# shenyunhang/JTSM

Hardware: AMD Instinct MI355X
Metric: images/sec training, R50-FPN JTSM panoptic, 2x1024x1024, 1/2/4/8 GPU (higher is better)
Workload: dtype bf16x3; 1 GPU; BASELINE configs[2]: JTSM panoptic R50-FPN, 2 x 3x1024x1024 per GPU, 2000 proposals + 1024 superpixels per image; MIL + 4 OICR + 2 mask heads + sem-seg; fwd + bwd + gradient exchange + SGD; 100% of proposals jittered copies of 40 rectangles per image; global_batch=2, parallelism=dp1, foreground_rois_last_step=281

## Files before the change

include/jtsm_hip.h:

```cpp
#ifndef JTSM_HIP_H_
#define JTSM_HIP_H_

#include <stddef.h>
#include <stdint.h>

#ifdef __cplusplus
extern "C" {
#endif

#define JTSM_OK 0
#define JTSM_EINVAL (-1)
#define JTSM_ELAUNCH (-2)
#define JTSM_ENODEV (-3)

#define JTSM_NCHW 0
#define JTSM_NHWC 1

const char* jtsm_last_error(void);
const char* jtsm_version(void);
int jtsm_device_count(void);

void* jtsm_event_create(void);
int jtsm_event_record(void* event, void* stream);
int jtsm_event_elapsed_ms(void* start, void* stop, float* ms);
// ... 73 lines not shown
                                        int sampling_ratio, int layout, void* workspace, size_t workspace_bytes,
                                        void* stream);
int jtsm_moi_pool_forward_f16(const uint16_t* input, const uint16_t* rois, const int32_t* oh_labels,
                              const int32_t* superpixels, uint16_t* output, int32_t* argmax, void* workspace,
                              size_t workspace_bytes, int B, int C, int H, int W, int M, int L, int Hs, int Ws,
                              float spatial_scale, int pooled_h, int pooled_w, int layout, void* stream);
int jtsm_moi_pool_backward_f16(const uint16_t* grad, const uint16_t* rois, const int32_t* argmax, uint16_t* grad_input,
                               void* workspace, size_t workspace_bytes, int B, int C, int H, int W, int M, int pooled_h,
                               int pooled_w, int layout, void* stream);

size_t jtsm_moi_pool_levels_workspace_bytes(int B, const int* H, const int* W, int nlevels, int M, int L);
int jtsm_moi_pool_forward_levels_f32(const float* const* inputs, const int* H, const int* W,
                                     const float* scales, int nlevels, const float* rois,
                                     const int32_t* roi_level, const int32_t* oh_labels,
                                     const int32_t* superpixels, float* output, int32_t* argmax,
                                     void* workspace, int B, int C, int M, int L, int Hs, int Ws,
                                     int pooled_h, int pooled_w, void* stream);
size_t jtsm_moi_pool_backward_levels_workspace_bytes(const int* H, const int* W, int nlevels, int B, int M);
int jtsm_moi_pool_backward_levels_f32(const float* grad, const float* rois, const int32_t* roi_level,
                                      const int32_t* argmax, float* const* grad_inputs, const int* H,
                                      const int* W, const float* scales, int nlevels, int B, int C, int M,
                                      int pooled_h, int pooled_w, int accumulate, void* workspace,
                                      size_t workspace_bytes, void* stream);

int jtsm_moi_mask_f32(const float* rois, const int32_t* oh_labels, const int32_t* superpixels,
                      int32_t* mois, void* workspace, int B, int H, int W, int M, int L, int Hs,
                      int Ws, float spatial_scale, void* stream);


typedef struct jtsm_conv_shape {
  int batch, in_h, in_w, in_c;
  int out_c;
  int kernel_h, kernel_w;
  int stride, pad, dilation;
} jtsm_conv_shape;

int jtsm_conv_out_size(const jtsm_conv_shape* s, int* out_h, int* out_w);
size_t jtsm_conv_workspace_bytes(const jtsm_conv_shape* s, int backward_data);
int jtsm_conv_plan(const jtsm_conv_shape* s, int role, int has_kscale, int* kernel, int* tile_m,
                   int* tile_n, int* splits);

int jtsm_conv2d_forward_f32(const float* x, const float* w, float* y, const jtsm_conv_shape* s,
                            const float* scale, const float* bias, const float* residual,
                            int relu, void* workspace, size_t workspace_bytes, void* stream);
int jtsm_conv2d_backward_data_f32(const float* dy, const float* w, float* dx,
                                  const jtsm_conv_shape* s, const float* kscale,
// ... 210 lines not shown

int jtsm_roi_align_forward_level_f32(const float* input, const float* rois,
                                     const int32_t* roi_level, int level, float* output, int B,
                                     int C, int H, int W, int M, float spatial_scale, int pooled_h,
                                     int pooled_w, int sampling_ratio, int aligned, void* stream);
int jtsm_roi_align_backward_level_f32(const float* grad, const float* rois,
                                      const int32_t* roi_level, int level, float* grad_input, int B,
                                      int C, int H, int W, int M, float spatial_scale, int pooled_h,
                                      int pooled_w, int sampling_ratio, int aligned, void* stream);
int jtsm_roi_align_rotated_forward_level_f32(const float* input, const float* rois, const int32_t* roi_level,
                                             int level, float* output, int B, int C, int H, int W, int M,
                                             float spatial_scale, int pooled_h, int pooled_w, int sampling_ratio,
                                             void* stream);
int jtsm_roi_align_rotated_backward_level_f32(const float* grad, const float* rois, const int32_t* roi_level,
                                              int level, float* grad_input, int B, int C, int H, int W, int M,
                                              float spatial_scale, int pooled_h, int pooled_w, int sampling_ratio,
                                              int accumulate, void* stream);
size_t jtsm_roi_align_backward_levels_workspace_bytes(const int* H, const int* W, int nlevels, int B, int C, int M);
int jtsm_roi_align_backward_levels_f32(const float* grad, const float* rois, const int32_t* roi_level,
                                       float* const* grad_inputs, const int* H, const int* W, const float* scales,
                                       int nlevels, int B, int C, int M, int pooled_h, int pooled_w, int sampling_ratio,
                                       int aligned, int accumulate, void* workspace, size_t workspace_bytes,
                                       void* stream);
int jtsm_moi_pool_forward_level_f32(const float* input, const float* rois, const int32_t* roi_level,
                                    int level, const int32_t* oh_labels, const int32_t* superpixels,
                                    float* output, int32_t* argmax, void* workspace, int B, int C,
                                    int H, int W, int M, int L, int Hs, int Ws, float spatial_scale,
                                    int pooled_h, int pooled_w, void* stream);
int jtsm_moi_pool_backward_level_f32(const float* grad, const float* rois, const int32_t* roi_level,
                                     int level, const int32_t* argmax, float* grad_input, int B, int C,
                                     int H, int W, int M, int pooled_h, int pooled_w, void* stream);


size_t jtsm_group_norm_workspace_bytes(int N, long HW, int C);
int jtsm_group_norm_forward_f32(const float* x, const float* gamma, const float* beta, float* y,
                                float* mean, float* rstd, void* workspace, int N, long HW, int C, int G,
                                float eps, int relu, void* stream);
int jtsm_group_norm_backward_f32(const float* x, const float* dy, const float* gamma, const float* beta,
                                 const float* mean, const float* rstd, float* dx, uint16_t* dx_hi,
                                 uint16_t* dx_lo, float* dgamma, float* dbeta, void* workspace, int N, long HW,
                                 int C, int G, int relu, void* stream);
int jtsm_upsample_bilinear2x_forward_f32(const float* x, float* y, uint16_t* y_hi, uint16_t* y_lo, int N, int H,
                                         int W, int C, void* stream);
int jtsm_upsample_bilinear2x_backward_f32(const float* gy, float* gx, int N, int H, int W, int C,
                                          void* stream);

// ... 78 lines not shown
```

jtsm_amd/csrc/moi_pool.hip:

```cpp
#include <algorithm>
#include <cfloat>

#include "common.h"

namespace jtsm {
namespace {

#pragma clang fp contract(off)

struct IBox { int b, x0, y0, x1, y1; };

__device__ __forceinline__ IBox round_box(const float* __restrict__ roi, float scale) {
#pragma clang fp contract(off)
  IBox r;
  r.b = (int)roi[0];
  r.x0 = (int)roundf(roi[1] * scale);
  r.y0 = (int)roundf(roi[2] * scale);
  r.x1 = (int)roundf(roi[3] * scale);
  r.y1 = (int)roundf(roi[4] * scale);
  return r;
}

__device__ __forceinline__ int clampi(int v, int lo, int hi) { return min(max(v, lo), hi); }

// ... 1273 lines not shown
static bool moi_bwd_events(hipEvent_t* fork, hipEvent_t* join) {
  static hipEvent_t ev[16][2] = {};
  int dev = 0;
  if (hipGetDevice(&dev) != hipSuccess || dev < 0 || dev >= 16) return false;
  for (int k = 0; k < 2; ++k)
    if (!ev[dev][k] && hipEventCreateWithFlags(&ev[dev][k], hipEventDisableTiming) != hipSuccess) return false;
  *fork = ev[dev][0];
  *join = ev[dev][1];
  return true;
}

static long census_tiles(const int* H, const int* W, int nlevels, int B) {
  long n = 0;
  for (int l = 0; l < nlevels; ++l) n += (long)B * ceil_div(W[l], kTile) * ceil_div(H[l], kTileY);
  return n;
}

size_t jtsm_moi_pool_backward_levels_workspace_bytes(const int* H, const int* W, int nlevels, int B, int M) {
  if (nlevels <= 0 || nlevels > kMaxLevels || B <= 0 || M <= 0 || !H || !W) return 0;
  return (((size_t)nlevels * B * ((size_t)M + 1) + 6 * (size_t)census_tiles(H, W, nlevels, B) + 8) * sizeof(int) + 15) &
         ~(size_t)15;
}

int jtsm_moi_pool_backward_levels_f32(const float* grad, const float* rois, const int32_t* roi_level,
                                      const int32_t* argmax, float* const* grad_inputs, const int* H, const int* W,
                                      const float* scales, int nlevels, int B, int C, int M, int pooled_h, int pooled_w,
                                      int accumulate, void* workspace, size_t workspace_bytes, void* stream) {
  JTSM_REQUIRE(nlevels > 0 && nlevels <= kMaxLevels && grad_inputs && H && W, "moi_pool levels backward: bad level table");
  JTSM_REQUIRE(B >= 0 && C >= 0 && M >= 0 && pooled_h > 0 && pooled_w > 0 && C % 4 == 0,
               "moi_pool levels backward: bad sizes (C %% 4 must be 0)");
  hipStream_t st = as_stream(stream);
  MoiLevels lv = {};
  bool all = true;
  for (int l = 0; l < nlevels; ++l) {
    lv.gin[l] = grad_inputs[l]; lv.H[l] = H[l]; lv.W[l] = W[l];
    lv.scale[l] = scales ? scales[l] : 0.f;
    all = all && grad_inputs[l] != nullptr;
  }
  bool small_maps = true;
  for (int l = 0; l < nlevels; ++l) small_maps = small_maps && (unsigned long long)H[l] * W[l] * W[l] < 0xFFFFFFFFull;
  const bool tiled = scales && workspace && all && small_maps && C % 256 == 0 && M > 0 && B > 0;
  if (tiled) {
    JTSM_REQUIRE(grad && rois && roi_level && argmax, "moi_pool levels backward: null pointer");
    const size_t need = jtsm_moi_pool_backward_levels_workspace_bytes(H, W, nlevels, B, M);
    JTSM_REQUIRE(workspace_bytes >= need && ((uintptr_t)workspace & 3) == 0,
                 "moi_pool levels backward: workspace of %zu bytes needed", need);
    int* lists = reinterpret_cast<int*>(workspace);
    int* counts = lists + (size_t)nlevels * B * M;
    int* census = counts + (size_t)nlevels * B;
    const int ntile = (int)census_tiles(H, W, nlevels, B);
    int* plan = census + ntile;
    hipLaunchKernelGGL(moi_roi_lists_kernel, dim3(nlevels * B), dim3(256), 0, st, rois, roi_level, M, B, lists, counts);
    MoiTiles tl = {};
    int blocks = 0;
    for (int l = 0; l < nlevels; ++l) {
      tl.first[l] = blocks;
      tl.tiles_x[l] = ceil_div(W[l], kTile);
      tl.tiles_y[l] = ceil_div(H[l], kTileY);
      blocks += B * tl.tiles_x[l] * tl.tiles_y[l];
    }
    tl.first[nlevels] = blocks;
    JTSM_CHECK_HIP(hipMemsetAsync(census, 0, (size_t)ntile * sizeof(int), st));
    hipLaunchKernelGGL(moi_tile_census_kernel, dim3(ceil_div(M, 256)), dim3(256), 0, st, lv, tl, rois, roi_level, M, nlevels,
                       pooled_h, pooled_w, census);
    int* tile_order = plan + 2 + 4 * (size_t)ntile;
    hipLaunchKernelGGL(tile_plan_kernel, dim3(1), dim3(1024), 0, st, census, ntile, plan, moi_heavy_min(), 4, tile_order);
    hipStream_t side = moi_bwd_side_stream();
    hipEvent_t fork = nullptr, join = nullptr;
    if (side && moi_bwd_events(&fork, &join)) {
      JTSM_CHECK_HIP(hipEventRecord(fork, st));
      JTSM_CHECK_HIP(hipStreamWaitEvent(side, fork, 0));
    } else {
      side = st;
    }
    hipLaunchKernelGGL(moi_pool_bwd_busy, dim3(256), dim3(1024), (size_t)kCopies * kQuad * kQuad * 256 * sizeof(float), side,
                       lv, tl, grad, rois, argmax, C, M, pooled_h, pooled_w, B, lists, counts, nlevels, plan, accumulate);
    hipLaunchKernelGGL(moi_pool_bwd_tiled, dim3(blocks, C / 256), dim3(256), kTile * kTile * 256 * sizeof(float), st, lv, tl,
                       grad, rois, argmax, C, M, pooled_h, pooled_w, B, lists, counts, nlevels, plan, census, moi_heavy_min(),
                       accumulate, tile_order);
    if (side != st) {
      JTSM_CHECK_HIP(hipEventRecord(join, side));
      JTSM_CHECK_HIP(hipStreamWaitEvent(st, join, 0));
    }
    hipLaunchKernelGGL(moi_pool_bwd_levels, dim3(std::min(ceil_div((long)M * pooled_h * pooled_w, 4), 8192)), dim3(256), 0,
                       st, lv, grad, rois, argmax, C, M, pooled_h * pooled_w, roi_level, nlevels, plan, kCensusLimit);
    JTSM_CHECK_LAUNCH("moi_pool backward levels (tiled)");
    return JTSM_OK;
  }
  for (int l = 0; l < nlevels; ++l) {
    if (!grad_inputs[l] || accumulate) continue;
    JTSM_CHECK_HIP(hipMemsetAsync(grad_inputs[l], 0, (size_t)B * H[l] * W[l] * C * sizeof(float), st));
  }
  if ((long)M * C == 0) return JTSM_OK;
  JTSM_REQUIRE(grad && rois && roi_level && argmax, "moi_pool levels backward: null pointer");
  for (int l = 0; l < nlevels; ++l)
    JTSM_REQUIRE(grad_inputs[l], "moi_pool levels backward: every level needs a gradient buffer");
  const int nbins = pooled_h * pooled_w;
  hipLaunchKernelGGL(moi_pool_bwd_levels, dim3(std::min(ceil_div((long)M * nbins, 4), 8192)), dim3(256), 0, st, lv, grad,
                     rois, argmax, C, M, nbins, roi_level, nlevels, (const int*)nullptr, 0);
  JTSM_CHECK_LAUNCH("moi_pool backward levels");
  return JTSM_OK;
}

}
```

jtsm_amd/csrc/roi_align.hip:

```cpp
#include <cstdlib>
#include <type_traits>

#include "common.h"
#include "roi_geometry.h"

namespace jtsm {
namespace {

#pragma clang fp contract(off)

template <typename T, int VEC> struct VecOf;
template <> struct VecOf<float, 4> { using type = float4; };
template <> struct VecOf<float, 1> { using type = float; };
template <> struct VecOf<double, 2> { using type = double2; };
template <> struct VecOf<double, 1> { using type = double; };

template <typename T, int VEC>
__device__ __forceinline__ void load_vec(const T* p, T (&v)[VEC]) {
  using V = typename VecOf<T, VEC>::type;
  const V x = *reinterpret_cast<const V*>(p);
  const T* e = reinterpret_cast<const T*>(&x);
#pragma unroll
  for (int i = 0; i < VEC; ++i) v[i] = e[i];
}
// ... 582 lines not shown
  } else {
    JTSM_REQUIRE(!roi_level, "roi_align: per-level filtering needs the NHWC layout");
    const long total = (long)M * C * PH * PW;
    const int blocks = (int)((total + 255) / 256 < 8192 ? (total + 255) / 256 : 8192);
    hipLaunchKernelGGL((align_fwd_nchw<T, ROT>), dim3(blocks), dim3(256), 0, st, in, rois, out, C,
                       H, W, total, scale, PH, PW, sr, aligned);
  }
  JTSM_CHECK_LAUNCH("roi_align forward");
  return JTSM_OK;
}

static size_t align_gather_head_bytes(int ntile, int C) {
  return ((size_t)ntile * (1 + C / 64) * sizeof(int) + 4 * sizeof(int) + 15) & ~(size_t)15;
}
static size_t align_gather_bytes(int ntile, int C, int M) {
  return align_gather_head_bytes(ntile, C) + (size_t)M * (sizeof(int4) + sizeof(int));
}
struct AsyncScratch {
  void* p = nullptr;
  hipStream_t st = nullptr;
  ~AsyncScratch() { if (p) (void)hipFreeAsync(p, st); }
};

static int align_backward_gather(const float* grad, const float* rois, AlignLevels& lv, int B, int C, int M, int PH,
                                 int PW, int sr, int aligned, const int* roi_level, hipStream_t st, bool accumulate = false,
                                 void* workspace = nullptr, size_t workspace_bytes = 0) {
  int ntile = 0;
  for (int l = 0; l < lv.n; ++l) {
    lv.tiles_x[l] = ceil_div(lv.W[l], kTile);
    lv.tiles_y[l] = ceil_div(lv.H[l], kTile);
    lv.first_tile[l] = ntile;
    ntile += B * lv.tiles_x[l] * lv.tiles_y[l];
  }
  lv.first_tile[lv.n] = ntile;
  const size_t need = align_gather_bytes(ntile, C, M);
  AsyncScratch own;
  own.st = st;
  if (workspace) {
    JTSM_REQUIRE(workspace_bytes >= need && ((uintptr_t)workspace & 15) == 0,
                 "roi_align backward: workspace of %zu bytes (16-byte aligned) needed, got %zu", need, workspace_bytes);
  } else {
    JTSM_CHECK_HIP(hipMallocAsync(&own.p, need, st));
  }
  for (int l = 0; l < lv.n && !accumulate; ++l)
    JTSM_CHECK_HIP(hipMemsetAsync(lv.gin[l], 0, (size_t)B * lv.H[l] * lv.W[l] * C * sizeof(float), st));
  int* census = reinterpret_cast<int*>(workspace ? workspace : own.p);
  const int fan = C / 64;
  const size_t head = align_gather_head_bytes(ntile, C);
  JTSM_CHECK_HIP(hipMemsetAsync(census, 0, (size_t)ntile * sizeof(int), st));
  int* plan = census + ntile;
  int4* reach = reinterpret_cast<int4*>(reinterpret_cast<char*>(census) + head);
  int* meta = reinterpret_cast<int*>(reach + M);
  hipLaunchKernelGGL(align_census_kernel, dim3(ceil_div(M, 256)), dim3(256), 0, st, rois, M, PH, PW, sr, aligned,
                     roi_level, lv, census, reach, meta);
  hipLaunchKernelGGL(tile_plan_kernel, dim3(1), dim3(1024), 0, st, census, ntile, plan, 1, fan);
  hipLaunchKernelGGL((align_bwd_gather<8, 1>), dim3(std::min(ntile * fan, 512)), dim3(256), 0, st, grad, rois, lv, C, M, PH,
                     PW, sr, aligned, plan, census_limit(), fan, reach, meta, accumulate ? 1 : 0);
  constexpr int V = WideVec<float>::value;
  const int blocks = ceil_div((long)M * PH * PW, 4);
  if (C % V == 0 && ((uintptr_t)grad % (V * sizeof(float))) == 0)
    hipLaunchKernelGGL((align_bwd_nhwc_levels<V>), dim3(blocks), dim3(256), 0, st, grad, rois, lv, C, M, PH, PW, sr, aligned,
                       roi_level, plan, census_limit());
  else
    hipLaunchKernelGGL((align_bwd_nhwc_levels<1>), dim3(blocks), dim3(256), 0, st, grad, rois, lv, C, M, PH, PW, sr, aligned,
                       roi_level, plan, census_limit());
  JTSM_CHECK_LAUNCH("roi_align backward (gather + census)");
  return JTSM_OK;
}

template <typename T, bool ROT>
int launch_backward(const T* grad, const T* rois, T* gin, int B, int C, int H, int W, int M,
                    T scale, int PH, int PW, int sr, int aligned, int layout, void* stream,
                    const int* roi_level = nullptr, int level = 0, bool accumulate = false) {
  JTSM_REQUIRE(B >= 0 && C >= 0 && H >= 0 && W >= 0 && M >= 0 && PH > 0 && PW > 0,
               "roi_align backward: negative size");
  JTSM_REQUIRE(layout == JTSM_NCHW || layout == JTSM_NHWC, "roi_align: unknown layout %d", layout);
  hipStream_t st = as_stream(stream);
  const size_t in_elems = (size_t)B * C * H * W;
  if (in_elems == 0) return JTSM_OK;
  JTSM_REQUIRE(gin, "roi_align backward: null grad_input");
// ... 366 lines not shown
                                             int level, float* output, int B, int C, int H, int W, int M,
                                             float spatial_scale, int pooled_h, int pooled_w, int sampling_ratio,
                                             void* stream) {
  JTSM_REQUIRE(roi_level || M == 0, "roi_align_rotated level: null roi_level");
  return launch_forward<float, true>(input, rois, output, B, C, H, W, M, spatial_scale, pooled_h, pooled_w,
                                     sampling_ratio, 1, JTSM_NHWC, stream, roi_level, level);
}
int jtsm_roi_align_rotated_backward_level_f32(const float* grad, const float* rois, const int32_t* roi_level,
                                              int level, float* grad_input, int B, int C, int H, int W, int M,
                                              float spatial_scale, int pooled_h, int pooled_w, int sampling_ratio,
                                              int accumulate, void* stream) {
  JTSM_REQUIRE(roi_level || M == 0, "roi_align_rotated level: null roi_level");
  return launch_backward<float, true>(grad, rois, grad_input, B, C, H, W, M, spatial_scale, pooled_h, pooled_w,
                                      sampling_ratio, 1, JTSM_NHWC, stream, roi_level, level, accumulate != 0);
}

size_t jtsm_roi_align_backward_levels_workspace_bytes(const int* H, const int* W, int nlevels, int B, int C, int M) {
  if (!H || !W || nlevels <= 0 || B <= 0 || C <= 0 || M < 0) return 0;
  long ntile = 0;
  for (int l = 0; l < nlevels; ++l) ntile += (long)B * ceil_div(W[l], kTile) * ceil_div(H[l], kTile);
  return align_gather_bytes((int)ntile, C, M);
}

int jtsm_roi_align_backward_levels_f32(const float* grad, const float* rois, const int32_t* roi_level,
                                       float* const* grad_inputs, const int* H, const int* W, const float* scales,
                                       int nlevels, int B, int C, int M, int pooled_h, int pooled_w, int sampling_ratio,
                                       int aligned, int accumulate, void* workspace, size_t workspace_bytes,
                                       void* stream) {
  JTSM_REQUIRE(nlevels > 0 && nlevels <= kAlignLevels && grad_inputs && H && W && scales,
               "roi_align levels: bad level table");
  JTSM_REQUIRE(B >= 0 && C >= 0 && M >= 0 && pooled_h > 0 && pooled_w > 0, "roi_align levels: negative size");
  JTSM_REQUIRE(roi_level || M == 0, "roi_align levels: null roi_level");
  hipStream_t st = as_stream(stream);
  const bool gather = C % 64 == 0 && C > 0 && B > 0 && grad && rois && pooled_w <= kMaxBins && pooled_h <= kMaxBins &&
                      (long)M * pooled_h * pooled_w >= 8192 && (long)M * pooled_h * pooled_w < (1L << 30);
  if (gather) {
    AlignLevels lv = {};
    lv.n = 0;
    for (int l = 0; l < nlevels; ++l) {
      if (!grad_inputs[l]) continue;
      JTSM_REQUIRE(H[l] > 0 && W[l] > 0, "roi_align levels: empty map");
      const int k = lv.n++;
      lv.gin[k] = grad_inputs[l]; lv.H[k] = H[l]; lv.W[k] = W[l]; lv.scale[k] = scales[l]; lv.level_id[k] = l;
    }
    if (lv.n == 0) return JTSM_OK;
    return align_backward_gather(grad, rois, lv, B, C, M, pooled_h, pooled_w, sampling_ratio, aligned, roi_level, st,
                                 accumulate != 0, workspace, workspace_bytes);
  }
  for (int l = 0; l < nlevels; ++l) {
    if (!grad_inputs[l]) continue;
    const int rc = launch_backward<float, false>(grad, rois, grad_inputs[l], B, C, H[l], W[l], M, scales[l], pooled_h,
                                                 pooled_w, sampling_ratio, aligned, JTSM_NHWC, stream, roi_level, l,
                                                 accumulate != 0);
    if (rc) return rc;
  }
  return JTSM_OK;
}

int jtsm_roi_sample_table_f32(const float* rois, int rotated, int M, int H, int W,
                              float spatial_scale, int pooled_h, int pooled_w, int sampling_ratio,
                              int aligned, int* grid, int* pos, float* w, int cap, void* stream) {
  JTSM_REQUIRE(M >= 0 && cap > 0 && pooled_h > 0 && pooled_w > 0, "sample_table: bad sizes");
  if (M == 0) return JTSM_OK;
  JTSM_REQUIRE(rois && grid && pos && w, "sample_table: null pointer");
  const long total = (long)M * cap;
  const int blocks = ceil_div(total, 256);
  if (rotated)
    hipLaunchKernelGGL((sample_table_kernel<float, true>), dim3(blocks), dim3(256), 0,
                       as_stream(stream), rois, M, H, W, spatial_scale, pooled_h, pooled_w,
                       sampling_ratio, 1, grid, pos, w, cap);
  else
    hipLaunchKernelGGL((sample_table_kernel<float, false>), dim3(blocks), dim3(256), 0,
                       as_stream(stream), rois, M, H, W, spatial_scale, pooled_h, pooled_w,
                       sampling_ratio, aligned, grid, pos, w, cap);
  JTSM_CHECK_LAUNCH("roi_sample_table");
  return JTSM_OK;
}

int jtsm_sp_mask_targets_f32(const float* rois, const int32_t* oh_row, const int32_t* img_of, const int32_t* oh_labels,
// ... 53 lines not shown
```

jtsm_amd/modeling/poolers.py:

```python
import math
from typing import List

import ctypes as C

import torch
from torch import nn
from torch.autograd import Function
from torch.autograd.function import once_differentiable

from .. import _lib as L
from ..layers import grad_fan
from ..layers.mining import MAX_IMAGES, pooler_rois_levels
from ..layers.moi_pool import MOIPool
from ..layers.roi_align import ROIAlign
from ..layers.roi_align_rotated import ROIAlignRotated
from ..layers.roi_loop_pool import ROILoopPool
from ..layers.wrappers import cat

CL = torch.channels_last


def assign_boxes_to_levels(box_lists, min_level, max_level, canonical_box_size, canonical_level):
    box_sizes = torch.sqrt(cat([boxes.area() for boxes in box_lists]))
    level_assignments = torch.floor(canonical_level + torch.log2(box_sizes / canonical_box_size + 1e-8))
    level_assignments = torch.clamp(torch.nan_to_num(level_assignments, nan=float(min_level)), min=min_level,
                                    max=max_level)
    return level_assignments.to(torch.int64) - min_level


def convert_boxes_to_pooler_format(box_lists):
    def fmt_box_list(box_tensor, batch_index):
        repeated_index = torch.full((len(box_tensor), 1), batch_index, dtype=box_tensor.dtype,
                                    device=box_tensor.device)
        return cat((repeated_index, box_tensor), dim=1)

    return cat([fmt_box_list(box_list.tensor, i) for i, box_list in enumerate(box_lists)], dim=0)


def _feat(x):
    L.require_gpu(x)
    if x.dtype != torch.float32:
        raise RuntimeError("jtsm_amd multi-level pooling is float32, got %s" % x.dtype)
    return x.contiguous(memory_format=CL)


class _AlignLevels(Function):
    @staticmethod
    def forward(ctx, rois, roi_level, res, sampling_ratio, aligned, scales, fans, *feats):
        ctx.fans = list(fans) if fans is not None else [None] * len(feats)
        rotated = aligned == "rotated"
        if rois.shape[1] != (6 if rotated else 5):
            raise RuntimeError("pooler rois must be (M, %d), got %s" % (6 if rotated else 5, tuple(rois.shape)))
        feats = [_feat(f) for f in feats]
        M, C = rois.shape[0], feats[0].shape[1]
        out = torch.empty((M, C, res, res), dtype=torch.float32, device=rois.device, memory_format=CL)
        for lvl, (f, sc) in enumerate(zip(feats, scales)):
            B, _, H, W = f.shape
            L.note_bytes(4.0 * (out.numel() / len(feats) + f.numel() + rois.numel()))
            if rotated:
                L.check(L.lib().jtsm_roi_align_rotated_forward_level_f32(
                    L.ptr(f), L.ptr(rois), L.ptr(roi_level), lvl, L.ptr(out), B, C, H, W, M, sc, res, res,
                    sampling_ratio, L.stream()), "roi_align_rotated_forward_level")
                continue
            L.check(L.lib().jtsm_roi_align_forward_level_f32(
                L.ptr(f), L.ptr(rois), L.ptr(roi_level), lvl, L.ptr(out), B, C, H, W, M, sc, res, res,
                sampling_ratio, int(aligned), L.stream()), "roi_align_forward_level")
        ctx.save_for_backward(rois, roi_level)
        ctx.cfg = (res, sampling_ratio, aligned, scales, [tuple(f.shape) for f in feats])
        return out

    @staticmethod
    @once_differentiable
    def backward(ctx, g):
        rois, roi_level = ctx.saved_tensors
        res, sampling_ratio, aligned, scales, shapes = ctx.cfg
        g = g.contiguous(memory_format=CL)
        nl = len(shapes)
        B, Cc = shapes[0][0], shapes[0][1]
# ... 2 lines not shown
        accumulate = any(wanted) and all(s is not None for s, w in zip(sinks, wanted) if w)
        grads = [(sinks[lvl] if accumulate else torch.empty(shapes[lvl], dtype=torch.float32, device=g.device,
                                                            memory_format=CL)) if wanted[lvl] else None
                 for lvl in range(nl)]
        if aligned == "rotated":
            for lvl in range(nl):
                if grads[lvl] is None:
                    continue
                L.note_bytes(4.0 * (g.numel() / nl + grads[lvl].numel() + rois.numel()))
                L.check(L.lib().jtsm_roi_align_rotated_backward_level_f32(
                    L.ptr(g), L.ptr(rois), L.ptr(roi_level), lvl, L.ptr(grads[lvl]), B, Cc, shapes[lvl][2],
                    shapes[lvl][3], rois.shape[0], scales[lvl], res, res, sampling_ratio, int(accumulate),
                    L.stream()), "roi_align_rotated_backward_level")
            if accumulate:
                return (None,) * (7 + nl)
            grads = [None if grad_fan.offer(ctx.fans[lvl], grads[lvl]) else grads[lvl] for lvl in range(nl)]
            return (None, None, None, None, None, None, None, *grads)
        Hs = (C.c_int * nl)(*[sh[2] for sh in shapes])
        Ws = (C.c_int * nl)(*[sh[3] for sh in shapes])
        sc = (C.c_float * nl)(*[float(x) for x in scales])
        ptrs = (C.c_void_p * nl)(*[(t.data_ptr() if t is not None else None) for t in grads])
        L.note_bytes(4.0 * (g.numel() + sum(t.numel() for t in grads if t is not None) + rois.numel()))
        lib = L.lib()
        ws = torch.empty(max(lib.jtsm_roi_align_backward_levels_workspace_bytes(Hs, Ws, nl, B, Cc, rois.shape[0]), 16),
                         dtype=torch.uint8, device=g.device)
        L.check(lib.jtsm_roi_align_backward_levels_f32(
            L.ptr(g), L.ptr(rois), L.ptr(roi_level), ptrs, Hs, Ws, sc, nl, B, Cc, rois.shape[0], res, res,
            sampling_ratio, int(aligned), int(accumulate), L.ptr(ws), ws.numel(), L.stream()),
            "roi_align_backward_levels")
        if accumulate:
            return (None,) * (7 + nl)
        grads = [None if grad_fan.offer(ctx.fans[lvl], grads[lvl]) else grads[lvl] for lvl in range(nl)]
        return (None, None, None, None, None, None, None, *grads)


class _MOILevels(Function):

    @staticmethod
    def forward(ctx, rois, roi_level, res, scales, oh_labels, superpixels, fans, *feats):
        ctx.fans = list(fans) if fans is not None else [None] * len(feats)
        feats = [_feat(f) for f in feats]
        M, Cc = rois.shape[0], feats[0].shape[1]
        Lw = oh_labels.shape[1]
        nl = len(feats)
        B = feats[0].shape[0]
        out = torch.empty((M, Cc, res, res), dtype=torch.float32, device=rois.device, memory_format=CL)
        arg = torch.empty((M, Cc, res, res), dtype=torch.int32, device=rois.device, memory_format=CL)
        lib = L.lib()
        Hs = (C.c_int * nl)(*[f.shape[2] for f in feats])
        Ws = (C.c_int * nl)(*[f.shape[3] for f in feats])
        sc = (C.c_float * nl)(*[float(x) for x in scales])
        ptrs = (C.c_void_p * nl)(*[f.data_ptr() for f in feats])
        ws = torch.empty(lib.jtsm_moi_pool_levels_workspace_bytes(B, Hs, Ws, nl, M, Lw), dtype=torch.uint8,
                         device=rois.device)
        L.note_bytes(4.0 * (sum(f.numel() for f in feats) + oh_labels.numel() + superpixels.numel() + 2 * out.numel()))
        L.check(lib.jtsm_moi_pool_forward_levels_f32(
            ptrs, Hs, Ws, sc, nl, L.ptr(rois), L.ptr(roi_level), L.ptr(oh_labels), L.ptr(superpixels), L.ptr(out),
            L.ptr(arg), L.ptr(ws), B, Cc, M, Lw, superpixels.shape[1], superpixels.shape[2], res, res, L.stream()),
            "moi_pool_forward_levels")
        ctx.save_for_backward(rois, roi_level, arg)
        ctx.cfg = (res, [tuple(f.shape) for f in feats], [float(x) for x in scales])
        ctx.mark_non_differentiable(arg)
        ctx.set_materialize_grads(False)
        return out, arg

    @staticmethod
    @once_differentiable
    def backward(ctx, g, _ga=None):
        if g is None:
            return (None,) * (7 + len(ctx.cfg[1]))
        rois, roi_level, arg = ctx.saved_tensors
        res, shapes, scales = ctx.cfg
        g = g.contiguous(memory_format=CL)
        nl = len(shapes)
        B, Cc = shapes[0][0], shapes[0][1]
        wanted = [bool(ctx.needs_input_grad[7 + lvl]) for lvl in range(nl)]
        sinks = [grad_fan.target(ctx.fans[lvl], shapes[lvl], g.device) for lvl in range(nl)]
        accumulate = all(wanted) and all(s is not None for s in sinks)
        grads = sinks if accumulate else [torch.empty(shape, dtype=torch.float32, device=g.device, memory_format=CL)
                                          for shape in shapes]
        Hs = (C.c_int * nl)(*[sh[2] for sh in shapes])
        Ws = (C.c_int * nl)(*[sh[3] for sh in shapes])
        ptrs = (C.c_void_p * nl)(*[t.data_ptr() for t in grads])
        sc = (C.c_float * nl)(*scales)
        lib = L.lib()
        ws = torch.empty(max(lib.jtsm_moi_pool_backward_levels_workspace_bytes(Hs, Ws, nl, B, rois.shape[0]), 16),
                         dtype=torch.uint8, device=g.device)
        L.note_bytes(4.0 * (2 * g.numel() + sum(t.numel() for t in grads)))
        L.check(lib.jtsm_moi_pool_backward_levels_f32(
            L.ptr(g), L.ptr(rois), L.ptr(roi_level), L.ptr(arg), ptrs, Hs, Ws, sc, nl, B, Cc, rois.shape[0], res, res,
            int(accumulate), L.ptr(ws), ws.numel(), L.stream()), "moi_pool_backward_levels")
        if accumulate:
            return (None,) * (7 + nl)
        grads = [gi if wanted[lvl] else None for lvl, gi in enumerate(grads)]
        grads = [None if grad_fan.offer(ctx.fans[lvl], grads[lvl]) else grads[lvl] for lvl in range(nl)]
        return (None, None, None, None, None, None, None, *grads)


def moi_label_inputs(oh_labels_list, superpixels):
    sp = superpixels.tensor if hasattr(superpixels, "tensor") else superpixels
    sp = sp.to(torch.int32).contiguous()
    if isinstance(oh_labels_list, torch.Tensor):
        return oh_labels_list.to(torch.int32).contiguous(), sp
    max_len = max(l.size(1) for l in oh_labels_list)
    labels = cat([l.to(torch.int32) if l.size(1) == max_len else
                  torch.nn.functional.pad(l.to(torch.int32), (0, max_len - l.size(1))) for l in oh_labels_list])
    return labels.contiguous(), sp


class ROIPooler(nn.Module):
    def __init__(self, output_size, scales, sampling_ratio, pooler_type, canonical_box_size=224,
                 canonical_level=4):
        super().__init__()
        if isinstance(output_size, int):
# ... 93 lines not shown
```

Measured before the change: 95.90 images/sec.

## Build pooler backward tile plans during forward and reuse them in backward

Splits the ROI-align and MoI-pool multi-level backward into a prepare phase (ROI lists, tile census, tile plan) and a consume phase. The prepare kernels now launch during forward, write into a persistent workspace kept on the autograd context, and backward skips rebuilding the plan. This moves small serial kernels, including a single-block planning kernel, off the backward critical path and avoids a workspace allocation there. The cost is extra memory held from forward to backward, plus extra work in forward when a backward never runs.

```diff
diff --git a/include/jtsm_hip.h b/include/jtsm_hip.h
--- a/include/jtsm_hip.h
+++ b/include/jtsm_hip.h
@@ -119,6 +119,15 @@
                                       const int* W, const float* scales, int nlevels, int B, int C, int M,
                                       int pooled_h, int pooled_w, int accumulate, void* workspace,
                                       size_t workspace_bytes, void* stream);
+size_t jtsm_moi_pool_backward_prep_workspace_bytes(const int* H, const int* W, int nlevels, int B, int M);
+int jtsm_moi_pool_backward_prepare(const float* rois, const int32_t* roi_level, const int* H, const int* W,
+                                   const float* scales, int nlevels, int B, int M, int pooled_h, int pooled_w,
+                                   void* prep, size_t prep_bytes, void* stream);
+int jtsm_moi_pool_backward_levels_prepared_f32(const float* grad, const float* rois, const int32_t* roi_level,
+                                               const int32_t* argmax, float* const* grad_inputs, const int* H,
+                                               const int* W, const float* scales, int nlevels, int B, int C, int M,
+                                               int pooled_h, int pooled_w, int accumulate, const void* prep,
+                                               size_t prep_bytes, void* stream);
 
 int jtsm_moi_mask_f32(const float* rois, const int32_t* oh_labels, const int32_t* superpixels,
                       int32_t* mois, void* workspace, int B, int H, int W, int M, int L, int Hs,
@@ -375,6 +384,15 @@
                                        int nlevels, int B, int C, int M, int pooled_h, int pooled_w, int sampling_ratio,
                                        int aligned, int accumulate, void* workspace, size_t workspace_bytes,
                                        void* stream);
+size_t jtsm_roi_align_backward_prep_workspace_bytes(const int* H, const int* W, int nlevels, int B, int C, int M);
+int jtsm_roi_align_backward_prepare(const float* rois, const int32_t* roi_level, const int* H, const int* W,
+                                    const float* scales, int nlevels, int B, int C, int M, int pooled_h, int pooled_w,
+                                    int sampling_ratio, int aligned, void* prep, size_t prep_bytes, void* stream);
+int jtsm_roi_align_backward_levels_prepared_f32(const float* grad, const float* rois, const int32_t* roi_level,
+                                                float* const* grad_inputs, const int* H, const int* W,
+                                                const float* scales, int nlevels, int B, int C, int M, int pooled_h,
+                                                int pooled_w, int sampling_ratio, int aligned, int accumulate,
+                                                const void* prep, size_t prep_bytes, void* stream);
 int jtsm_moi_pool_forward_level_f32(const float* input, const float* rois, const int32_t* roi_level,
                                     int level, const int32_t* oh_labels, const int32_t* superpixels,
                                     float* output, int32_t* argmax, void* workspace, int B, int C,
diff --git a/jtsm_amd/csrc/moi_pool.hip b/jtsm_amd/csrc/moi_pool.hip
--- a/jtsm_amd/csrc/moi_pool.hip
+++ b/jtsm_amd/csrc/moi_pool.hip
@@ -1319,10 +1319,68 @@
          ~(size_t)15;
 }
 
-int jtsm_moi_pool_backward_levels_f32(const float* grad, const float* rois, const int32_t* roi_level,
-                                      const int32_t* argmax, float* const* grad_inputs, const int* H, const int* W,
-                                      const float* scales, int nlevels, int B, int C, int M, int pooled_h, int pooled_w,
-                                      int accumulate, void* workspace, size_t workspace_bytes, void* stream) {
+struct MoiPrep {
+  int* lists; int* counts; int* census; int* plan; int* tile_order;
+  int ntile;
+  MoiTiles tl;
+};
+static MoiPrep moi_prep_carve(void* workspace, const int* H, const int* W, int nlevels, int B, int M) {
+  MoiPrep p = {};
+  p.lists = reinterpret_cast<int*>(workspace);
+  p.counts = p.lists + (size_t)nlevels * B * M;
+  p.census = p.counts + (size_t)nlevels * B;
+  p.ntile = (int)census_tiles(H, W, nlevels, B);
+  p.plan = p.census + p.ntile;
+  p.tile_order = p.plan + 2 + 4 * (size_t)p.ntile;
+  int blocks = 0;
+  for (int l = 0; l < nlevels; ++l) {
+    p.tl.first[l] = blocks;
+    p.tl.tiles_x[l] = ceil_div(W[l], kTile);
+    p.tl.tiles_y[l] = ceil_div(H[l], kTileY);
+    blocks += B * p.tl.tiles_x[l] * p.tl.tiles_y[l];
+  }
+  p.tl.first[nlevels] = blocks;
+  return p;
+}
+static bool moi_gather_geometry_ok(const int* H, const int* W, const float* scales, int nlevels, int B, int M) {
+  bool small_maps = true;
+  for (int l = 0; l < nlevels; ++l) small_maps = small_maps && (unsigned long long)H[l] * W[l] * W[l] < 0xFFFFFFFFull;
+  return scales && small_maps && M > 0 && B > 0;
+}
+static int moi_prepare_launch(const MoiPrep& p, const MoiLevels& lv, const float* rois, const int32_t* roi_level, int nlevels,
+                              int B, int M, int pooled_h, int pooled_w, hipStream_t st) {
+  hipLaunchKernelGGL(moi_roi_lists_kernel, dim3(nlevels * B), dim3(256), 0, st, rois, roi_level, M, B, p.lists, p.counts);
+  JTSM_CHECK_HIP(hipMemsetAsync(p.census, 0, (size_t)p.ntile * sizeof(int), st));
+  hipLaunchKernelGGL(moi_tile_census_kernel, dim3(ceil_div(M, 256)), dim3(256), 0, st, lv, p.tl, rois, roi_level, M, nlevels,
+                     pooled_h, pooled_w, p.census);
+  hipLaunchKernelGGL(tile_plan_kernel, dim3(1), dim3(1024), 0, st, p.census, p.ntile, p.plan, moi_heavy_min(), 4, p.tile_order);
+  JTSM_CHECK_LAUNCH("moi_pool backward prepare");
+  return JTSM_OK;
+}
+
+size_t jtsm_moi_pool_backward_prep_workspace_bytes(const int* H, const int* W, int nlevels, int B, int M) {
+  return jtsm_moi_pool_backward_levels_workspace_bytes(H, W, nlevels, B, M);
+}
+
+int jtsm_moi_pool_backward_prepare(const float* rois, const int32_t* roi_level, const int* H, const int* W,
+                                   const float* scales, int nlevels, int B, int M, int pooled_h, int pooled_w, void* prep,
+                                   size_t prep_bytes, void* stream) {
+  JTSM_REQUIRE(nlevels > 0 && nlevels <= kMaxLevels && H && W, "moi_pool backward prepare: bad level table");
+  JTSM_REQUIRE(B >= 0 && M >= 0 && pooled_h > 0 && pooled_w > 0, "moi_pool backward prepare: bad sizes");
+  if (!moi_gather_geometry_ok(H, W, scales, nlevels, B, M)) return JTSM_OK;
+  JTSM_REQUIRE(rois && roi_level && prep, "moi_pool backward prepare: null pointer");
+  const size_t need = jtsm_moi_pool_backward_levels_workspace_bytes(H, W, nlevels, B, M);
+  JTSM_REQUIRE(prep_bytes >= need && ((uintptr_t)prep & 3) == 0, "moi_pool backward prepare: workspace of %zu bytes needed", need);
+  MoiLevels lv = {};
+  for (int l = 0; l < nlevels; ++l) { lv.H[l] = H[l]; lv.W[l] = W[l]; lv.scale[l] = scales[l]; }
+  return moi_prepare_launch(moi_prep_carve(prep, H, W, nlevels, B, M), lv, rois, roi_level, nlevels, B, M, pooled_h, pooled_w,
+                            as_stream(stream));
+}
+
+static int moi_backward_levels_impl(const float* grad, const float* rois, const int32_t* roi_level,
+                                    const int32_t* argmax, float* const* grad_inputs, const int* H, const int* W,
+                                    const float* scales, int nlevels, int B, int C, int M, int pooled_h, int pooled_w,
+                                    int accumulate, void* workspace, size_t workspace_bytes, void* stream, bool prepared) {
   JTSM_REQUIRE(nlevels > 0 && nlevels <= kMaxLevels && grad_inputs && H && W, "moi_pool levels backward: bad level table");
   JTSM_REQUIRE(B >= 0 && C >= 0 && M >= 0 && pooled_h > 0 && pooled_w > 0 && C % 4 == 0,
                "moi_pool levels backward: bad sizes (C %% 4 must be 0)");
@@ -1334,34 +1392,21 @@
     lv.scale[l] = scales ? scales[l] : 0.f;
     all = all && grad_inputs[l] != nullptr;
   }
-  bool small_maps = true;
-  for (int l = 0; l < nlevels; ++l) small_maps = small_maps && (unsigned long long)H[l] * W[l] * W[l] < 0xFFFFFFFFull;
-  const bool tiled = scales && workspace && all && small_maps && C % 256 == 0 && M > 0 && B > 0;
+  const bool tiled = workspace && all && C % 256 == 0 && moi_gather_geometry_ok(H, W, scales, nlevels, B, M);
   if (tiled) {
     JTSM_REQUIRE(grad && rois && roi_level && argmax, "moi_pool levels backward: null pointer");
     const size_t need = jtsm_moi_pool_backward_levels_workspace_bytes(H, W, nlevels, B, M);
     JTSM_REQUIRE(workspace_bytes >= need && ((uintptr_t)workspace & 3) == 0,
                  "moi_pool levels backward: workspace of %zu bytes needed", need);
-    int* lists = reinterpret_cast<int*>(workspace);
-    int* counts = lists + (size_t)nlevels * B * M;
-    int* census = counts + (size_t)nlevels * B;
-    const int ntile = (int)census_tiles(H, W, nlevels, B);
-    int* plan = census + ntile;
-    hipLaunchKernelGGL(moi_roi_lists_kernel, dim3(nlevels * B), dim3(256), 0, st, rois, roi_level, M, B, lists, counts);
-    MoiTiles tl = {};
-    int blocks = 0;
-    for (int l = 0; l < nlevels; ++l) {
-      tl.first[l] = blocks;
-      tl.tiles_x[l] = ceil_div(W[l], kTile);
-      tl.tiles_y[l] = ceil_div(H[l], kTileY);
-      blocks += B * tl.tiles_x[l] * tl.tiles_y[l];
-    }
-    tl.first[nlevels] = blocks;
-    JTSM_CHECK_HIP(hipMemsetAsync(census, 0, (size_t)ntile * sizeof(int), st));
-    hipLaunchKernelGGL(moi_tile_census_kernel, dim3(ceil_div(M, 256)), dim3(256), 0, st, lv, tl, rois, roi_level, M, nlevels,
-                       pooled_h, pooled_w, census);
-    int* tile_order = plan + 2 + 4 * (size_t)ntile;
-    hipLaunchKernelGGL(tile_plan_kernel, dim3(1), dim3(1024), 0, st, census, ntile, plan, moi_heavy_min(), 4, tile_order);
+    const MoiPrep pp = moi_prep_carve(workspace, H, W, nlevels, B, M);
+    if (!prepared) {
+      const int rc = moi_prepare_launch(pp, lv, rois, roi_level, nlevels, B, M, pooled_h, pooled_w, st);
+      if (rc) return rc;
+    }
+    const int* lists = pp.lists; const int* counts = pp.counts; const int* census = pp.census; const int* plan = pp.plan;
+    const int* tile_order = pp.tile_order;
+    const MoiTiles& tl = pp.tl;
+    const int blocks = tl.first[nlevels];
     hipStream_t side = moi_bwd_side_stream();
     hipEvent_t fork = nullptr, join = nullptr;
     if (side && moi_bwd_events(&fork, &join)) {
@@ -1399,4 +1444,22 @@
   return JTSM_OK;
 }
 
-}
+int jtsm_moi_pool_backward_levels_f32(const float* grad, const float* rois, const int32_t* roi_level,
+                                      const int32_t* argmax, float* const* grad_inputs, const int* H, const int* W,
+                                      const float* scales, int nlevels, int B, int C, int M, int pooled_h, int pooled_w,
+                                      int accumulate, void* workspace, size_t workspace_bytes, void* stream) {
+  return moi_backward_levels_impl(grad, rois, roi_level, argmax, grad_inputs, H, W, scales, nlevels, B, C, M, pooled_h,
+                                  pooled_w, accumulate, workspace, workspace_bytes, stream, false);
+}
+
+int jtsm_moi_pool_backward_levels_prepared_f32(const float* grad, const float* rois, const int32_t* roi_level,
+                                               const int32_t* argmax, float* const* grad_inputs, const int* H, const int* W,
+                                               const float* scales, int nlevels, int B, int C, int M, int pooled_h,
+                                               int pooled_w, int accumulate, const void* prep, size_t prep_bytes,
+                                               void* stream) {
+  JTSM_REQUIRE(prep, "moi_pool levels backward (prepared): null preparation");
+  return moi_backward_levels_impl(grad, rois, roi_level, argmax, grad_inputs, H, W, scales, nlevels, B, C, M, pooled_h,
+                                  pooled_w, accumulate, const_cast<void*>(prep), prep_bytes, stream, true);
+}
+
+}
diff --git a/jtsm_amd/csrc/roi_align.hip b/jtsm_amd/csrc/roi_align.hip
--- a/jtsm_amd/csrc/roi_align.hip
+++ b/jtsm_amd/csrc/roi_align.hip
@@ -628,9 +628,7 @@
   ~AsyncScratch() { if (p) (void)hipFreeAsync(p, st); }
 };
 
-static int align_backward_gather(const float* grad, const float* rois, AlignLevels& lv, int B, int C, int M, int PH,
-                                 int PW, int sr, int aligned, const int* roi_level, hipStream_t st, bool accumulate = false,
-                                 void* workspace = nullptr, size_t workspace_bytes = 0) {
+static int align_tile_table(AlignLevels& lv, int B) {
   int ntile = 0;
   for (int l = 0; l < lv.n; ++l) {
     lv.tiles_x[l] = ceil_div(lv.W[l], kTile);
@@ -639,6 +637,31 @@
     ntile += B * lv.tiles_x[l] * lv.tiles_y[l];
   }
   lv.first_tile[lv.n] = ntile;
+  return ntile;
+}
+struct AlignPrep { int* census; int* plan; int4* reach; int* meta; };
+static AlignPrep align_prep_carve(void* ws, int ntile, int C, int M) {
+  AlignPrep p;
+  p.census = reinterpret_cast<int*>(ws);
+  p.plan = p.census + ntile;
+  p.reach = reinterpret_cast<int4*>(reinterpret_cast<char*>(ws) + align_gather_head_bytes(ntile, C));
+  p.meta = reinterpret_cast<int*>(p.reach + M);
+  return p;
+}
+static int align_prepare_launch(const AlignPrep& p, const float* rois, const AlignLevels& lv, int ntile, int C, int M, int PH,
+                                int PW, int sr, int aligned, const int* roi_level, hipStream_t st) {
+  JTSM_CHECK_HIP(hipMemsetAsync(p.census, 0, (size_t)ntile * sizeof(int), st));
+  hipLaunchKernelGGL(align_census_kernel, dim3(ceil_div(M, 256)), dim3(256), 0, st, rois, M, PH, PW, sr, aligned,
+                     roi_level, lv, p.census, p.reach, p.meta);
+  hipLaunchKernelGGL(tile_plan_kernel, dim3(1), dim3(1024), 0, st, p.census, ntile, p.plan, 1, C / 64);
+  JTSM_CHECK_LAUNCH("roi_align backward prepare");
+  return JTSM_OK;
+}
+
+static int align_backward_gather(const float* grad, const float* rois, AlignLevels& lv, int B, int C, int M, int PH,
+                                 int PW, int sr, int aligned, const int* roi_level, hipStream_t st, bool accumulate = false,
+                                 void* workspace = nullptr, size_t workspace_bytes = 0, bool prepared = false) {
+  const int ntile = align_tile_table(lv, B);
   const size_t need = align_gather_bytes(ntile, C, M);
   AsyncScratch own;
   own.st = st;
@@ -646,22 +669,20 @@
     JTSM_REQUIRE(workspace_bytes >= need && ((uintptr_t)workspace & 15) == 0,
                  "roi_align backward: workspace of %zu bytes (16-byte aligned) needed, got %zu", need, workspace_bytes);
   } else {
+    JTSM_REQUIRE(!prepared, "roi_align backward: null preparation");
     JTSM_CHECK_HIP(hipMallocAsync(&own.p, need, st));
   }
   for (int l = 0; l < lv.n && !accumulate; ++l)
     JTSM_CHECK_HIP(hipMemsetAsync(lv.gin[l], 0, (size_t)B * lv.H[l] * lv.W[l] * C * sizeof(float), st));
-  int* census = reinterpret_cast<int*>(workspace ? workspace : own.p);
+  const AlignPrep pp = align_prep_carve(workspace ? workspace : own.p, ntile, C, M);
   const int fan = C / 64;
-  const size_t head = align_gather_head_bytes(ntile, C);
-  JTSM_CHECK_HIP(hipMemsetAsync(census, 0, (size_t)ntile * sizeof(int), st));
-  int* plan = census + ntile;
-  int4* reach = reinterpret_cast<int4*>(reinterpret_cast<char*>(census) + head);
-  int* meta = reinterpret_cast<int*>(reach + M);
-  hipLaunchKernelGGL(align_census_kernel, dim3(ceil_div(M, 256)), dim3(256), 0, st, rois, M, PH, PW, sr, aligned,
-                     roi_level, lv, census, reach, meta);
-  hipLaunchKernelGGL(tile_plan_kernel, dim3(1), dim3(1024), 0, st, census, ntile, plan, 1, fan);
+  if (!prepared) {
+    const int rc = align_prepare_launch(pp, rois, lv, ntile, C, M, PH, PW, sr, aligned, roi_level, st);
+    if (rc) return rc;
+  }
+  const int* plan = pp.plan;
   hipLaunchKernelGGL((align_bwd_gather<8, 1>), dim3(std::min(ntile * fan, 512)), dim3(256), 0, st, grad, rois, lv, C, M, PH,
-                     PW, sr, aligned, plan, census_limit(), fan, reach, meta, accumulate ? 1 : 0);
+                     PW, sr, aligned, plan, census_limit(), fan, pp.reach, pp.meta, accumulate ? 1 : 0);
   constexpr int V = WideVec<float>::value;
   const int blocks = ceil_div((long)M * PH * PW, 4);
   if (C % V == 0 && ((uintptr_t)grad % (V * sizeof(float))) == 0)
@@ -1074,30 +1095,37 @@
   return align_gather_bytes((int)ntile, C, M);
 }
 
-int jtsm_roi_align_backward_levels_f32(const float* grad, const float* rois, const int32_t* roi_level,
-                                       float* const* grad_inputs, const int* H, const int* W, const float* scales,
-                                       int nlevels, int B, int C, int M, int pooled_h, int pooled_w, int sampling_ratio,
-                                       int aligned, int accumulate, void* workspace, size_t workspace_bytes,
-                                       void* stream) {
+static bool align_levels_gather_ok(int B, int C, int M, int pooled_h, int pooled_w) {
+  return C % 64 == 0 && C > 0 && B > 0 && pooled_w <= kMaxBins && pooled_h <= kMaxBins &&
+         (long)M * pooled_h * pooled_w >= 8192 && (long)M * pooled_h * pooled_w < (1L << 30);
+}
+
+static int align_backward_levels_impl(const float* grad, const float* rois, const int32_t* roi_level,
+                                      float* const* grad_inputs, const int* H, const int* W, const float* scales,
+                                      int nlevels, int B, int C, int M, int pooled_h, int pooled_w, int sampling_ratio,
+                                      int aligned, int accumulate, void* workspace, size_t workspace_bytes,
+                                      void* stream, bool prepared) {
   JTSM_REQUIRE(nlevels > 0 && nlevels <= kAlignLevels && grad_inputs && H && W && scales,
                "roi_align levels: bad level table");
   JTSM_REQUIRE(B >= 0 && C >= 0 && M >= 0 && pooled_h > 0 && pooled_w > 0, "roi_align levels: negative size");
   JTSM_REQUIRE(roi_level || M == 0, "roi_align levels: null roi_level");
   hipStream_t st = as_stream(stream);
-  const bool gather = C % 64 == 0 && C > 0 && B > 0 && grad && rois && pooled_w <= kMaxBins && pooled_h <= kMaxBins &&
-                      (long)M * pooled_h * pooled_w >= 8192 && (long)M * pooled_h * pooled_w < (1L << 30);
+  const bool gather = grad && rois && align_levels_gather_ok(B, C, M, pooled_h, pooled_w);
   if (gather) {
     AlignLevels lv = {};
     lv.n = 0;
     for (int l = 0; l < nlevels; ++l) {
-      if (!grad_inputs[l]) continue;
+      if (!grad_inputs[l]) {
+        JTSM_REQUIRE(!prepared, "roi_align levels (prepared): every level needs a gradient buffer");
+        continue;
+      }
       JTSM_REQUIRE(H[l] > 0 && W[l] > 0, "roi_align levels: empty map");
       const int k = lv.n++;
       lv.gin[k] = grad_inputs[l]; lv.H[k] = H[l]; lv.W[k] = W[l]; lv.scale[k] = scales[l]; lv.level_id[k] = l;
     }
     if (lv.n == 0) return JTSM_OK;
     return align_backward_gather(grad, rois, lv, B, C, M, pooled_h, pooled_w, sampling_ratio, aligned, roi_level, st,
-                                 accumulate != 0, workspace, workspace_bytes);
+                                 accumulate != 0, workspace, workspace_bytes, prepared);
   }
   for (int l = 0; l < nlevels; ++l) {
     if (!grad_inputs[l]) continue;
@@ -1107,6 +1135,50 @@
     if (rc) return rc;
   }
   return JTSM_OK;
+}
+
+int jtsm_roi_align_backward_levels_f32(const float* grad, const float* rois, const int32_t* roi_level,
+                                       float* const* grad_inputs, const int* H, const int* W, const float* scales,
+                                       int nlevels, int B, int C, int M, int pooled_h, int pooled_w, int sampling_ratio,
+                                       int aligned, int accumulate, void* workspace, size_t workspace_bytes,
+                                       void* stream) {
+  return align_backward_levels_impl(grad, rois, roi_level, grad_inputs, H, W, scales, nlevels, B, C, M, pooled_h, pooled_w,
+                                    sampling_ratio, aligned, accumulate, workspace, workspace_bytes, stream, false);
+}
+
+size_t jtsm_roi_align_backward_prep_workspace_bytes(const int* H, const int* W, int nlevels, int B, int C, int M) {
+  return jtsm_roi_align_backward_levels_workspace_bytes(H, W, nlevels, B, C, M);
+}
+
+int jtsm_roi_align_backward_prepare(const float* rois, const int32_t* roi_level, const int* H, const int* W,
+                                    const float* scales, int nlevels, int B, int C, int M, int pooled_h, int pooled_w,
+                                    int sampling_ratio, int aligned, void* prep, size_t prep_bytes, void* stream) {
+  JTSM_REQUIRE(nlevels > 0 && nlevels <= kAlignLevels && H && W && scales, "roi_align backward prepare: bad level table");
+  JTSM_REQUIRE(B >= 0 && C >= 0 && M >= 0 && pooled_h > 0 && pooled_w > 0, "roi_align backward prepare: negative size");
+  if (!align_levels_gather_ok(B, C, M, pooled_h, pooled_w)) return JTSM_OK;
+  JTSM_REQUIRE(rois && roi_level && prep, "roi_align backward prepare: null pointer");
+  AlignLevels lv = {};
+  lv.n = nlevels;
+  for (int l = 0; l < nlevels; ++l) {
+    JTSM_REQUIRE(H[l] > 0 && W[l] > 0, "roi_align backward prepare: empty map");
+    lv.H[l] = H[l]; lv.W[l] = W[l]; lv.scale[l] = scales[l]; lv.level_id[l] = l;
+  }
+  const int ntile = align_tile_table(lv, B);
+  const size_t need = align_gather_bytes(ntile, C, M);
+  JTSM_REQUIRE(prep_bytes >= need && ((uintptr_t)prep & 15) == 0,
+               "roi_align backward prepare: workspace of %zu bytes (16-byte aligned) needed, got %zu", need, prep_bytes);
+  return align_prepare_launch(align_prep_carve(prep, ntile, C, M), rois, lv, ntile, C, M, pooled_h, pooled_w, sampling_ratio,
+                              aligned, roi_level, as_stream(stream));
+}
+
+int jtsm_roi_align_backward_levels_prepared_f32(const float* grad, const float* rois, const int32_t* roi_level,
+                                                float* const* grad_inputs, const int* H, const int* W,
+                                                const float* scales, int nlevels, int B, int C, int M, int pooled_h,
+                                                int pooled_w, int sampling_ratio, int aligned, int accumulate,
+                                                const void* prep, size_t prep_bytes, void* stream) {
+  JTSM_REQUIRE(prep, "roi_align levels (prepared): null preparation");
+  return align_backward_levels_impl(grad, rois, roi_level, grad_inputs, H, W, scales, nlevels, B, C, M, pooled_h, pooled_w,
+                                    sampling_ratio, aligned, accumulate, const_cast<void*>(prep), prep_bytes, stream, true);
 }
 
 int jtsm_roi_sample_table_f32(const float* rois, int rotated, int M, int H, int W,
diff --git a/jtsm_amd/modeling/poolers.py b/jtsm_amd/modeling/poolers.py
--- a/jtsm_amd/modeling/poolers.py
+++ b/jtsm_amd/modeling/poolers.py
@@ -1,7 +1,9 @@
 import math
+import os
 from typing import List
 
 import ctypes as C
+import ctypes as _ct
 
 import torch
 from torch import nn
@@ -18,6 +20,8 @@
 from ..layers.wrappers import cat
 
 CL = torch.channels_last
+
+POOL_PREP = os.environ.get("JTSM_POOL_PREP", "1") != "0"
 
 
 def assign_boxes_to_levels(box_lists, min_level, max_level, canonical_box_size, canonical_level):
@@ -54,6 +58,18 @@
         feats = [_feat(f) for f in feats]
         M, C = rois.shape[0], feats[0].shape[1]
         out = torch.empty((M, C, res, res), dtype=torch.float32, device=rois.device, memory_format=CL)
+        prep = None
+        if POOL_PREP and not rotated and M > 0 and all(ctx.needs_input_grad[7:7 + len(feats)]):
+            lib, nl, B = L.lib(), len(feats), feats[0].shape[0]
+            Hs = (_ct.c_int * nl)(*[f.shape[2] for f in feats])
+            Ws = (_ct.c_int * nl)(*[f.shape[3] for f in feats])
+            sc_ = (_ct.c_float * nl)(*[float(x) for x in scales])
+            nb = lib.jtsm_roi_align_backward_prep_workspace_bytes(Hs, Ws, nl, B, C, M)
+            prep = torch.empty(max(nb, 16), dtype=torch.uint8, device=rois.device)
+            L.check(lib.jtsm_roi_align_backward_prepare(
+                L.ptr(rois), L.ptr(roi_level), Hs, Ws, sc_, nl, B, C, M, res, res, sampling_ratio, int(aligned),
+                L.ptr(prep), prep.numel(), L.stream()), "roi_align_backward_prepare")
+        ctx.prep = prep
         for lvl, (f, sc) in enumerate(zip(feats, scales)):
             B, _, H, W = f.shape
             L.note_bytes(4.0 * (out.numel() / len(feats) + f.numel() + rois.numel()))
@@ -102,6 +118,16 @@
         ptrs = (C.c_void_p * nl)(*[(t.data_ptr() if t is not None else None) for t in grads])
         L.note_bytes(4.0 * (g.numel() + sum(t.numel() for t in grads if t is not None) + rois.numel()))
         lib = L.lib()
+        prep = getattr(ctx, "prep", None)
+        if prep is not None and all(wanted):
+            L.check(lib.jtsm_roi_align_backward_levels_prepared_f32(
+                L.ptr(g), L.ptr(rois), L.ptr(roi_level), ptrs, Hs, Ws, sc, nl, B, Cc, rois.shape[0], res, res,
+                sampling_ratio, int(aligned), int(accumulate), L.ptr(prep), prep.numel(), L.stream()),
+                "roi_align_backward_levels_prepared")
+            if accumulate:
+                return (None,) * (7 + nl)
+            grads = [None if grad_fan.offer(ctx.fans[lvl], grads[lvl]) else grads[lvl] for lvl in range(nl)]
+            return (None, None, None, None, None, None, None, *grads)
         ws = torch.empty(max(lib.jtsm_roi_align_backward_levels_workspace_bytes(Hs, Ws, nl, B, Cc, rois.shape[0]), 16),
                          dtype=torch.uint8, device=g.device)
         L.check(lib.jtsm_roi_align_backward_levels_f32(
@@ -133,6 +159,14 @@
         ptrs = (C.c_void_p * nl)(*[f.data_ptr() for f in feats])
         ws = torch.empty(lib.jtsm_moi_pool_levels_workspace_bytes(B, Hs, Ws, nl, M, Lw), dtype=torch.uint8,
                          device=rois.device)
+        prep = None
+        if POOL_PREP and M > 0 and any(ctx.needs_input_grad[7:7 + nl]):
+            nb = lib.jtsm_moi_pool_backward_prep_workspace_bytes(Hs, Ws, nl, B, M)
+            prep = torch.empty(max(nb, 16), dtype=torch.uint8, device=rois.device)
+            L.check(lib.jtsm_moi_pool_backward_prepare(
+                L.ptr(rois), L.ptr(roi_level), Hs, Ws, sc, nl, B, M, res, res, L.ptr(prep), prep.numel(), L.stream()),
+                "moi_pool_backward_prepare")
+        ctx.prep = prep
         L.note_bytes(4.0 * (sum(f.numel() for f in feats) + oh_labels.numel() + superpixels.numel() + 2 * out.numel()))
         L.check(lib.jtsm_moi_pool_forward_levels_f32(
             ptrs, Hs, Ws, sc, nl, L.ptr(rois), L.ptr(roi_level), L.ptr(oh_labels), L.ptr(superpixels), L.ptr(out),
@@ -164,12 +198,18 @@
         ptrs = (C.c_void_p * nl)(*[t.data_ptr() for t in grads])
         sc = (C.c_float * nl)(*scales)
         lib = L.lib()
-        ws = torch.empty(max(lib.jtsm_moi_pool_backward_levels_workspace_bytes(Hs, Ws, nl, B, rois.shape[0]), 16),
-                         dtype=torch.uint8, device=g.device)
+        prep = getattr(ctx, "prep", None)
         L.note_bytes(4.0 * (2 * g.numel() + sum(t.numel() for t in grads)))
-        L.check(lib.jtsm_moi_pool_backward_levels_f32(
-            L.ptr(g), L.ptr(rois), L.ptr(roi_level), L.ptr(arg), ptrs, Hs, Ws, sc, nl, B, Cc, rois.shape[0], res, res,
-            int(accumulate), L.ptr(ws), ws.numel(), L.stream()), "moi_pool_backward_levels")
+        if prep is not None:
+            L.check(lib.jtsm_moi_pool_backward_levels_prepared_f32(
+                L.ptr(g), L.ptr(rois), L.ptr(roi_level), L.ptr(arg), ptrs, Hs, Ws, sc, nl, B, Cc, rois.shape[0], res, res,
+                int(accumulate), L.ptr(prep), prep.numel(), L.stream()), "moi_pool_backward_levels_prepared")
+        else:
+            ws = torch.empty(max(lib.jtsm_moi_pool_backward_levels_workspace_bytes(Hs, Ws, nl, B, rois.shape[0]), 16),
+                             dtype=torch.uint8, device=g.device)
+            L.check(lib.jtsm_moi_pool_backward_levels_f32(
+                L.ptr(g), L.ptr(rois), L.ptr(roi_level), L.ptr(arg), ptrs, Hs, Ws, sc, nl, B, Cc, rois.shape[0], res, res,
+                int(accumulate), L.ptr(ws), ws.numel(), L.stream()), "moi_pool_backward_levels")
         if accumulate:
             return (None,) * (7 + nl)
         grads = [gi if wanted[lvl] else None for lvl, gi in enumerate(grads)]
```

Measured after the change: 95.91 images/sec, median of 3. Within noise of the previous version (+0.0%).
